# juliuspleunes4/TurboInfer

Measured on AMD Instinct MI355X. Metric: decode tokens/s/GPU, Llama-7B-shape INT4 @2048 ctx; % HBM-read roofline, higher is better.
Workload: dtype w4a16; 1 GPU; llama2-7b INT4 g128 decode, 1 stream(s)/GPU, KV 2048, replay at pos 2047; model=llama2-7b, global_batch=1, seq_len=2048, parallelism=replicas1 (request-sharded, no collectives)

## Files before the change

include/ti_hip.h:

```cpp
#ifndef TI_HIP_H
#define TI_HIP_H

#include <stddef.h>
#include <stdint.h>

#ifdef __cplusplus
extern "C" {
#endif

typedef void* ti_stream_t;

enum ti_status {
  TI_OK = 0,
  TI_ERR_ARG = 1,
  TI_ERR_HIP = 2,
  TI_ERR_UNSUPPORTED = 3,
  TI_ERR_NOMEM = 4,
  TI_ERR_NODEV = 5
};

const char* ti_last_error(void);

int ti_device_count(int* count);
int ti_init(int device);
// ... 111 lines not shown
                   int kv_heads, int head_dim, int splits, float* workspace, uint16_t* out,
                   ti_stream_t s);
int ti_attn_decode_packed(const float* q, const uint16_t* k_cache, const uint16_t* v_cache,
                          int64_t kv_stream_stride, int max_seq, const int32_t* pos, int M, int heads,
                          int kv_heads, int head_dim, int splits, float* workspace, uint16_t* out,
                          ti_stream_t s);
#ifndef TI_ATTN_MAX_PART_SPLITS
#define TI_ATTN_MAX_PART_SPLITS 8
#endif
int ti_attn_decode_partials(const float* q, const uint16_t* k_cache, const uint16_t* v_cache,
                            int64_t kv_stream_stride, int max_seq, const int32_t* pos, int M, int heads,
                            int kv_heads, int head_dim, int splits, uint16_t* part_o, float* part_ml,
                            ti_stream_t s);
int ti_attn_decode_f8(const float* q, const uint8_t* k_cache, const uint8_t* v_cache, int64_t kv_stream_stride,
                      int max_seq, const int32_t* pos, int M, int heads, int kv_heads, int head_dim, int splits,
                      float* workspace, uint16_t* out, ti_stream_t s);
int ti_attn_decode_packed_f8(const float* q, const uint8_t* k_cache, const uint8_t* v_cache,
                             int64_t kv_stream_stride, int max_seq, const int32_t* pos, int M, int heads,
                             int kv_heads, int head_dim, int splits, float* workspace, uint16_t* out,
                             ti_stream_t s);
int ti_attn_decode_partials_f8(const float* q, const uint8_t* k_cache, const uint8_t* v_cache,
                               int64_t kv_stream_stride, int max_seq, const int32_t* pos, int M, int heads,
                               int kv_heads, int head_dim, int splits, uint16_t* part_o, float* part_ml,
                               ti_stream_t s);
int ti_qkv_attn_partials(const void* tiles, const uint16_t* scales, int bits, const uint16_t* fx,
                         const float* ss_in, int n_ss, float eps, const float* rope_cs, const int32_t* pos,
                         uint16_t* k_cache, uint16_t* v_cache, int max_seq, int K, int heads, int kv_heads,
                         int head_dim, int splits, uint16_t* part_o, float* part_ml, void* xchg, ti_stream_t s);
size_t ti_qkv_attn_part_o_elems(int heads, int head_dim, int splits);
size_t ti_qkv_attn_part_ml_elems(int heads, int head_dim, int splits);
size_t ti_qkv_attn_xchg_bytes(int heads, int splits);
size_t ti_qkv_attn_error_offset(int heads, int splits);
int ti_qkv_attn_supported(int bits, int K, int heads, int kv_heads, int head_dim, int splits);
int ti_attn_prefill(const float* q, const uint16_t* k_cache, const uint16_t* v_cache, int max_seq,
                    const int32_t* pos, int M, int heads, int kv_heads, int head_dim, uint16_t* out,
                    ti_stream_t s);
int ti_attn_prefill_f8(const float* q, const uint8_t* k_cache, const uint8_t* v_cache, int max_seq,
                       const int32_t* pos, int M, int heads, int kv_heads, int head_dim, uint16_t* out,
                       ti_stream_t s);
size_t ti_attn_prefill_split_workspace_bytes(int M, int heads, int head_dim, int splits);
int ti_attn_prefill_split(const float* q, const uint16_t* k_cache, const uint16_t* v_cache, int max_seq,
                          const int32_t* pos, int M, int heads, int kv_heads, int head_dim, int splits,
                          float* workspace, uint16_t* out, ti_stream_t s);
int ti_attn_prefill_set_kernel(int mode);

int ti_gemm_kernel_name(int bits, int x_kind, int M, int N, int K, char* buf, int len);

uint64_t ti_gemm_onerow_epi_launches(void);

int ti_hbm_calibrate(size_t bytes, int reps, double* read_gbps, double* copy_gbps, ti_stream_t s);


typedef struct ti_step_args {
  const uint16_t* emb;
  float* h;
  int32_t hidden, M, vocab, in_stride, out_stride, placeholder_first;
  const int32_t* in_tokens;
  const int32_t* n_in;
  unsigned long long* argmax;
  int32_t* out_tokens;
  int32_t* pos;
  const int32_t* base_pos;
  const int32_t* step_ctr;
  const float* fold_w;
  uint16_t* fold_x;
  float* fold_ss;
// ... 57 lines not shown
```

turboinfer_amd/__init__.py:

```python
from __future__ import annotations

import ctypes as C
import os
import subprocess

import numpy as np

HERE = os.path.dirname(os.path.abspath(__file__))
ROOT = os.path.dirname(HERE)
LIB_PATH = os.environ.get("TI_LIB") or os.path.join(HERE, "lib", "libturboinfer_amd.so")

TI_OK = 0
X_F16, X_F32, X_F32_RMSNORM, X_F16_FOLDED, X_ATTN_SPLITS, X_F16_PACKED = 0, 1, 2, 3, 4, 5
ATTN_MAX_PART_SPLITS = 8
EPI_STORE_F32, EPI_STORE_F16, EPI_RESID_F32, EPI_SILU_MUL_F16, EPI_QKV_ROPE_KV, EPI_LOGITS_ARGMAX = range(6)
ARGMAX_SLOTS = 32
GEMM_MAX_ROWS = 1024
BITS_G32 = 32
BITS_AFF = 64
BITS_KV8 = 128
SCALE_GROUP, SCALE_TENSOR, SCALE_UNIT = 0, 1, 2
ROWS_CONCAT, ROWS_INTERLEAVE8 = 0, 1
(W_Q, W_K, W_V, W_O, W_GATE, W_UP, W_DOWN, W_LM_HEAD, V_ATTN_NORM, V_FFN_NORM, V_OUT_NORM, E_EMBED) = range(12)

# ... 40 lines not shown
                ("max_batch", C.c_int32), ("compat", C.c_int32), ("device", C.c_int32),
                ("attn_splits", C.c_int32)]


EXPORTED = [
    "ti_last_error", "ti_device_count", "ti_init", "ti_device_name", "ti_malloc", "ti_free", "ti_memcpy_h2d",
    "ti_memcpy_d2h", "ti_memcpy_d2d", "ti_memset", "ti_stream_create", "ti_stream_destroy", "ti_stream_sync",
    "ti_device_sync", "ti_event_create", "ti_event_destroy", "ti_event_record", "ti_event_elapsed_ms",
    "ti_wpack_tile_bytes", "ti_wpack_scale_bytes", "ti_wpack_host", "ti_wsynth_device", "ti_fill_uniform_f16",
    "ti_fill_uniform_f32", "ti_fill_kv_uniform", "ti_kv_copy_slots", "ti_gemm_wq_a16", "ti_gemm_lds_bytes", "ti_gemm_prepare",
    "ti_gemm_max_rows", "ti_gemm_packed_rows", "ti_gemm_packed_rows_for", "ti_gemm_tile_plan", "ti_rmsnorm_f16", "ti_rmsnorm_f16_packed", "ti_attn_decode_packed", "ti_attn_prefill", "ti_attn_prefill_set_kernel",
    "ti_attn_workspace_bytes", "ti_attn_decode", "ti_step_begin", "ti_matmul_f32", "ti_rms_norm_f32",
    "ti_rope_f32", "ti_silu_f32", "ti_relu_f32", "ti_add_f32", "ti_mul_f32", "ti_softmax_f32", "ti_attention_f32",
    "ti_argmax_f32", "ti_engine_create", "ti_engine_destroy", "ti_engine_get_stream", "ti_engine_memory", "ti_engine_set_tensor",
    "ti_engine_synth", "ti_engine_fill_kv", "ti_engine_generate", "ti_engine_step", "ti_engine_compat_step",
    "ti_engine_replay_prepare", "ti_engine_set_prefill", "ti_engine_replay_run", "ti_engine_sync", "ti_engine_last_tokens",
    "ti_engine_time_kernel", "ti_engine_stamp_steps", "ti_rope_table", "ti_sample_token", 
    "ti_gemm_grid", "ti_engine_set_fold",
    "ti_attn_decode_partials", "ti_sample_device", "ti_sample_step", "ti_engine_generate_sampled",
    "ti_engine_beam_search", "ti_engine_serve", 
    "ti_wpack_q_host", "ti_engine_set_tensor_q", "ti_sample_workspace_bytes", "ti_sample_device_ws",
    "ti_wpack_q1_host", "ti_engine_set_tensor_q1", "ti_epilogue_bytes",
    "ti_sample_step_ws", "ti_hbm_calibrate", "ti_gemm_kernel_name",
    "ti_gemm_fold_partials", "ti_engine_set_stop", "ti_engine_counters",
    "ti_qkv_attn_partials", "ti_qkv_attn_part_o_elems", "ti_qkv_attn_part_ml_elems", "ti_engine_set_qkv_attn",
    "ti_qkv_attn_xchg_bytes", "ti_qkv_attn_supported", "ti_qkv_attn_error_offset",
    "ti_logprob_rows", "ti_engine_score",
    "ti_attn_decode_f8", "ti_attn_decode_packed_f8", "ti_attn_decode_partials_f8", "ti_fill_kv_uniform_f8",
    "ti_attn_prefill_f8", "ti_engine_prefill_attn_name",
    "ti_engine_read_kv",
    "ti_attn_prefill_split", "ti_attn_prefill_split_workspace_bytes", "ti_lookahead_begin", "ti_lookahead_accept",
    "ti_engine_generate_lookahead",
    "ti_gemm_onerow_epi_launches",
]

_lib = None


def build(jobs: int = 8) -> None:
    subprocess.run(["make", "-s", "-C", ROOT, f"-j{jobs}", "all"], check=True)


def lib() -> C.CDLL:
    global _lib
    if _lib is None:
        if not os.path.exists(LIB_PATH):
            raise TiError(f"native library missing: {LIB_PATH} (run `make` or __graft_entry__.build())")
        L = C.CDLL(LIB_PATH)
        vp, i32, i64, u64, f32, sz = C.c_void_p, C.c_int, C.c_int64, C.c_uint64, C.c_float, C.c_size_t
        L.ti_last_error.restype = C.c_char_p
        L.ti_device_count.argtypes = [C.POINTER(C.c_int)]
        L.ti_init.argtypes = [i32]
        L.ti_device_name.argtypes = [i32, C.c_char_p, i32]
        L.ti_malloc.argtypes = [C.POINTER(vp), sz]
        L.ti_free.argtypes = [vp]
        for n in ("ti_memcpy_h2d", "ti_memcpy_d2h", "ti_memcpy_d2d"):
            getattr(L, n).argtypes = [vp, vp, sz, vp]
        L.ti_memset.argtypes = [vp, i32, sz, vp]
        L.ti_stream_sync.argtypes = [vp]
        L.ti_wpack_tile_bytes.argtypes = [i32, i32, i32]
        L.ti_wpack_tile_bytes.restype = sz
        L.ti_wpack_scale_bytes.argtypes = [i32, i32, i32]
        L.ti_wpack_scale_bytes.restype = sz
        L.ti_wpack_host.argtypes = [vp, i32, i32, i32, i32, i32, i32, i32, vp, vp]
        L.ti_wsynth_device.argtypes = [u64, C.c_uint32, i32, i32, i32, i32, i32, i32, vp, vp, vp]
        L.ti_fill_uniform_f16.argtypes = [u64, C.c_uint32, u64, f32, vp, vp]
# ... 67 lines not shown
            L.ti_qkv_attn_partials.argtypes = [vp, vp, i32, vp, vp, i32, f32, vp, vp, vp, vp, i32, i32, i32, i32,
                                               i32, i32, vp, vp, vp, vp]
            L.ti_qkv_attn_xchg_bytes.argtypes = [i32, i32]
            L.ti_qkv_attn_supported.argtypes = [i32, i32, i32, i32, i32, i32]
            L.ti_qkv_attn_xchg_bytes.restype = sz
            L.ti_qkv_attn_error_offset.argtypes = [i32, i32]
            L.ti_qkv_attn_error_offset.restype = sz
            L.ti_qkv_attn_part_o_elems.argtypes = [i32, i32, i32]
            L.ti_qkv_attn_part_o_elems.restype = sz
            L.ti_qkv_attn_part_ml_elems.argtypes = [i32, i32, i32]
            L.ti_qkv_attn_part_ml_elems.restype = sz
        if hasattr(L, "ti_engine_score"):
            L.ti_logprob_rows.argtypes = [vp, i32, i32, i32, vp, vp, vp, vp]
            L.ti_engine_score.argtypes = [vp, i32, vp, i32, i32, vp, vp, vp]
        if hasattr(L, "ti_attn_decode_f8"):
            for n in ("ti_attn_decode_f8", "ti_attn_decode_packed_f8", "ti_attn_decode_partials_f8"):
                getattr(L, n).argtypes = [vp, vp, vp, i64, i32, vp, i32, i32, i32, i32, i32, vp, vp, vp]
            L.ti_fill_kv_uniform_f8.argtypes = [u64, C.c_uint32, i32, i32, i32, i32, vp, vp]
            L.ti_engine_read_kv.argtypes = [vp, i32, i32, i32, i32, i32, vp]
        if hasattr(L, "ti_attn_prefill_f8"):
            L.ti_attn_prefill_f8.argtypes = [vp, vp, vp, i32, vp, i32, i32, i32, i32, vp, vp]
            L.ti_engine_prefill_attn_name.argtypes = [vp, i32, C.c_char_p, i32]
        if hasattr(L, "ti_engine_generate_lookahead"):
            L.ti_attn_prefill_split.argtypes = [vp, vp, vp, i32, vp, i32, i32, i32, i32, i32, vp, vp, vp]
            L.ti_attn_prefill_split_workspace_bytes.argtypes = [i32, i32, i32, i32]
            L.ti_attn_prefill_split_workspace_bytes.restype = sz
            L.ti_lookahead_begin.argtypes = [C.POINTER(LookaheadArgs), vp]
            L.ti_lookahead_accept.argtypes = [C.POINTER(LookaheadArgs), vp]
            L.ti_engine_generate_lookahead.argtypes = [vp, i32, vp, i32, i32, vp, i32, i32, i32, i32, vp,
                                                       C.POINTER(LookaheadStats)]
        if hasattr(L, "ti_gemm_onerow_epi_launches"):
            L.ti_gemm_onerow_epi_launches.argtypes = []
            L.ti_gemm_onerow_epi_launches.restype = u64
        L.ti_engine_compat_step.argtypes = [vp, i32, vp]
        L.ti_engine_replay_prepare.argtypes = [vp, i32, i32, i32]
        L.ti_engine_replay_run.argtypes = [vp, i32]
        L.ti_engine_sync.argtypes = [vp]
        L.ti_engine_last_tokens.argtypes = [vp, i32, vp]
        L.ti_engine_time_kernel.argtypes = [vp, i32, i32, i32, i32, C.POINTER(C.c_double), C.POINTER(C.c_double)]
        if hasattr(L, "ti_engine_stamp_steps"):
            L.ti_engine_stamp_steps.argtypes = [vp, i32, i32, vp, vp, C.POINTER(C.c_int)]
        L.ti_hbm_calibrate.argtypes = [sz, i32, C.POINTER(C.c_double), C.POINTER(C.c_double), vp]
        L.ti_gemm_kernel_name.argtypes = [i32, i32, i32, i32, i32, C.c_char_p, i32]
        L.ti_rope_table.argtypes = [vp, i32, i32, f32, vp]
        L.ti_sample_token.argtypes = [vp, i32, f32, i32, f32, f32, C.POINTER(C.c_int), C.POINTER(C.c_float)]
        _lib = L
    return _lib


def check(rc: int) -> None:
    if rc != TI_OK:
        raise TiError(f"ti error {rc}: {lib().ti_last_error().decode()}")


def device_count() -> int:
    n = C.c_int(0)
    check(lib().ti_device_count(C.byref(n)))
    return n.value


def init(device: int = 0) -> None:
    check(lib().ti_init(device))


def _ptr(a: np.ndarray) -> C.c_void_p:
    return C.c_void_p(a.ctypes.data)
# ... 311 lines not shown
```

turboinfer_amd/csrc/host/engine.cpp:

```cpp
#include <hip/hip_runtime.h>

#include <algorithm>
#include <atomic>
#include <cmath>
#include <queue>
#include <cstdio>
#include <cstdlib>
#include <cstring>
#include <map>
#include <utility>
#include <vector>

#include "ti_engine.h"
#include "ti_hip.h"

int ti_set_error(int code, const char* fmt, ...);
int ti_check_hip(hipError_t e, const char* what);

#define E_CHECK(expr, what)                                \
  do {                                                     \
    hipError_t _e = (expr);                                \
    if (_e != hipSuccess) return ti_check_hip(_e, what);   \
  } while (0)
#define TI_TRY(expr)                 \
// ... 1922 lines not shown
  if (!e || e->replay_M < 1 || steps < 1 || steps > 256 || cap < 1 || !info_out || !t_out || !n_launch)
    return ti_set_error(TI_ERR_ARG, "ti_engine_stamp_steps: call ti_engine_replay_prepare first; 1 <= steps <= 256, "
                        "cap >= 1");
  DeviceScope bind_(e);
  TI_TRY(ti_stream_sync(e->s));
  std::vector<int32_t> info, info2;
  TI_TRY(capture_stamped(e, 1, nullptr, {}, info, nullptr));
  const size_t n = info.size() / 3, nt = n * (size_t)steps;
  std::vector<size_t> offs(nt);
  size_t words = 0;
  for (size_t i = 0; i < nt; ++i) {
    offs[i] = words;
    words += (size_t)info[3 * (i % n) + 2] * kStampWords;
  }
  if (words == 0) return ti_set_error(TI_ERR_UNSUPPORTED, "ti_engine_stamp_steps: no stamped launch in the step");
  void* buf = nullptr;
  TI_TRY(ti_malloc(&buf, words * 8));
  unsigned long long* st = static_cast<unsigned long long*>(buf);
  hipGraphExec_t g = nullptr;
  int rc = capture_stamped(e, steps, st, offs, info2, &g);
  if (rc == TI_OK && (info2.size() != nt * 3 || !std::equal(info.begin(), info.end(), info2.begin())))
    rc = ti_set_error(TI_ERR_UNSUPPORTED, "ti_engine_stamp_steps: the two captures differ");
  std::vector<unsigned long long> h(words);
  for (int it = 0; rc == TI_OK && it < 2; ++it) {
    hipError_t he = hipMemsetAsync(st, 0, words * 8, e->s);
    if (he == hipSuccess) he = hipGraphLaunch(g, e->s);
    if (he == hipSuccess && it == 1) he = hipMemcpyAsync(h.data(), st, words * 8, hipMemcpyDeviceToHost, e->s);
    if (he == hipSuccess) he = hipStreamSynchronize(e->s);
    if (he != hipSuccess) rc = ti_check_hip(he, "ti_engine_stamp_steps: replay");
  }
  if (g) hipGraphExecDestroy(g);
  ti_free(buf);
  TI_TRY(rc);
  constexpr double kUs = 0.01;
  std::vector<double> acc(n * TI_STAMP_FIELDS, 0.0), first(nt, 0.0), last_end(nt, 0.0);
  for (size_t i = 0; i < nt; ++i) {
    const int wgs = info[3 * (i % n) + 2];
    if (wgs == 0) continue;
    unsigned long long f = ~0ull, le = 0, lent = 0;
    double wskew = 0.0;
    std::vector<unsigned long long> ends, cus;
    ends.reserve(wgs);
    double ph[6] = {0, 0, 0, 0, 0, 0}, sskew = 0.0;
    int sskew_n = 0;
    int phn[6] = {0, 0, 0, 0, 0, 0};
    for (int w = 0; w < wgs; ++w) {
      const unsigned long long* p = h.data() + offs[i] + (size_t)w * kStampWords;
      if (p[0]) {
        f = std::min(f, p[0]);
        lent = std::max(lent, p[0]);
      }
      if (p[15]) cus.push_back((p[15] & 0x7FFFFFFF00000000ull) | (p[15] & 0xFF00ull));
      unsigned long long smn = ~0ull, smx = 0;
      for (int k = 16; k < 24; ++k)
        if (p[k]) {
          smn = std::min(smn, p[k]);
          smx = std::max(smx, p[k]);
        }
      if (smx) {
        sskew += (double)(smx - smn);
        ++sskew_n;
      }
      unsigned long long mn = ~0ull, mx = 0;
      for (int k = 1; k <= 8; ++k)
        if (p[k]) {
          mn = std::min(mn, p[k]);
// ... 58 lines not shown
```

turboinfer_amd/csrc/kernels/qkv_attn.hip:

```cpp
#include <math.h>
#include <stdlib.h>

#include "attention_body.hpp"
#include "common.hpp"
#include "dequant.hpp"
#include "ti_hip.h"

namespace ti {

struct QkvAttnArgs {
  const u32x4* tiles;
  const uint16_t* scales;
  const uint16_t* fx;
  const float* ss;
  int n_ss;
  float eps;
  const float* rope_cs;
  const int32_t* pos;
  uint16_t* kc;
  uint16_t* vc;
  int max_seq, K, heads, kv_heads, kv_shift, splits, kv_tiles;
  int last_extra;
  float scale;
  uint16_t* part_o;
  float* part_ml;
  unsigned long long* xchg;
  unsigned long long* stamp;
  uint32_t* err;
  int drop;
};

constexpr int kQaWaves = 8, kQaThreads = kQaWaves * kWave;
#ifndef TI_QA_KV_RING
#define TI_QA_KV_RING 3
#endif
#ifndef TI_QA_ISSUE_BARRIER
#define TI_QA_ISSUE_BARRIER 0
#endif
#ifndef TI_QA_KVW_LATE
#define TI_QA_KVW_LATE 0
#endif
#ifndef TI_QA_KV_LATE
#define TI_QA_KV_LATE -1
#endif
constexpr int kQaSlot = 32;
constexpr int kQaMaxK = 4096;
constexpr int kQaMaxKv = 2;
constexpr unsigned kQaSpin = 1u << 16;

__device__ __forceinline__ float int4_x_prep_qa(f16x8& h) {
  const f16 s16 = (f16)0.0625f;
  h[2] *= s16; h[3] *= s16; h[6] *= s16; h[7] *= s16;
  const float lo = ((float)h[0] + (float)h[1]) + ((float)h[4] + (float)h[5]);
  const float hi = ((float)h[2] + (float)h[3]) + ((float)h[6] + (float)h[7]);
  return 1032.0f * lo + 1152.0f * hi;
}

__host__ __device__ inline int qa_kv_tile(int h, int s, int i, int heads, int splits, int kv_tiles) {
  const int j = h + heads * (splits - 1 - s) + heads * splits * i;
  return j < kv_tiles ? j : -1;
}

template <int BITS, int HD, int NQ, int NK>
__global__ __launch_bounds__(kQaThreads, 1) void qkv_attn_kernel(const QkvAttnArgs a) {
  const unsigned long long t_entry = stamp_now();
  constexpr int C = TileFmt<BITS>::kChunks;
  constexpr int QT = HD / 16;
  __shared__ __attribute__((aligned(16))) f16 xl[kQaMaxK + 8];
  __shared__ __attribute__((aligned(16))) uint16_t sl[1 + kQaMaxKv][kQaMaxK / 128][16];
  __shared__ __attribute__((aligned(16))) float corr[kQaMaxK / 128][16];
  __shared__ u32x4 sl_dummy;
  __shared__ float slab[1 + kQaMaxKv][kQaWaves][16];
  __shared__ float q_s[HD];
  __shared__ float s_m[kQaWaves], s_l[kQaWaves];
  __shared__ __attribute__((aligned(16))) float s_acc[kQaWaves][HD];

  const int tid = threadIdx.x, lane = tid & 63;
  const int wave = __builtin_amdgcn_readfirstlane(tid >> 6);
  const int S = a.splits, h = (int)blockIdx.x / S, s = (int)blockIdx.x % S;
  const int K = a.K, KT = K >> 7, K8 = K >> 3;
  const int qd = a.heads * HD, kvd = a.kv_heads * HD;
  const int kparts = S / QT, tq = s % QT, kp = s / QT;
  const int KTP = KT / kparts;
  int gk[kQaMaxKv], nkv = 0;
#pragma unroll
  for (int i = 0; i < kQaMaxKv; ++i) {
    const int j = qa_kv_tile(h, s, i, a.heads, S, a.kv_tiles);
    gk[i] = qd / 16 + (j >= 0 ? j : 0);
    nkv += j >= 0 ? 1 : 0;
  }
  const int gq = h * QT + tq;
  unsigned long long* my_slot = a.xchg + ((size_t)h * S + s) * kQaSlot;

  int zero;
  asm volatile("v_mov_b32 %0, 0" : "=v"(zero));
  const int p_v = a.pos[zero];
  const uint32_t gen_prev = ld_sc1_u32((const uint32_t*)(my_slot + (zero & 15)) + 1);
  const int n_scq = KTP * 2, n_sc = n_scq + nkv * KT * 2;
  u32x4 sc_reg;
  {
    const int ic = tid < n_sc ? tid : 0, r2 = ic - n_scq, ik = r2 >= KT * 2 ? 1 : 0;
    const int g = ic < n_scq ? gq : ik ? gk[1] : gk[0];
    const int piece = ic < n_scq ? kp * KTP * 2 + ic : r2 - ik * KT * 2;
    sc_reg = *((const u32x4*)(a.scales + (size_t)g * KT * 16) + piece);
  }
  const u32x4 xr0 = *(const u32x4*)(a.fx + 8 * (tid < K8 ? tid : K8 - 1));
  float ss4[4];
#pragma unroll
  for (int j = 0; j < 4; ++j) ss4[j] = a.ss[lane + 64 * j < a.n_ss ? lane + 64 * j : 0];
  asm volatile("" ::: "memory");
  if constexpr (HD == 128 && TI_QA_ISSUE_BARRIER) __builtin_amdgcn_s_barrier();
  u32x4 wq[NQ][C];
#pragma unroll
  for (int i = 0; i < NQ; ++i) {
    const u32x4* src = a.tiles + ((size_t)gq * KT + kp * KTP + wave + kQaWaves * i) * (kWave * C) + lane;
#pragma unroll
    for (int c = 0; c < C; ++c) wq[i][c] = *(src + c * kWave);
  }
  constexpr bool kKvwUniform = HD == 128;
  u32x4 wk[kQaMaxKv][NK][C];
  auto load_kv_weights = [&]() {
#pragma unroll
    for (int t = 0; t < kQaMaxKv; ++t)
#pragma unroll
      for (int i = 0; i < NK; ++i)
        if (kKvwUniform || t < nkv) {
          const u32x4* src = a.tiles + ((size_t)gk[t] * KT + wave + kQaWaves * i) * (kWave * C) + lane;
#pragma unroll
          for (int c = 0; c < C; ++c) wk[t][i][c] = __builtin_nontemporal_load(src + c * kWave);
        }
  };
  if constexpr (kKvwUniform && !TI_QA_KVW_LATE) load_kv_weights();
  asm volatile("" ::: "memory");
  u32x4 xr = xr0;
  if constexpr (kKvwUniform)
    asm volatile("" : "+v"(xr), "+v"(sc_reg), "+v"(ss4[0]), "+v"(ss4[1]), "+v"(ss4[2]), "+v"(ss4[3]));
  {
    f16x8 hx = __builtin_bit_cast(f16x8, xr);
    float part = 0.0f;
    if constexpr (BITS == 4) part = int4_x_prep_qa(hx);
    *(f16x8*)(xl + 8 * tid) = hx;
    if constexpr (BITS == 4) {
      part = group_sum<16>(part);
      if (tid < K8 && (lane & 15) == 0) corr[tid >> 4][0] = part;
    }
  }
  {
    const int r2 = tid - n_scq, ik = r2 >= KT * 2 ? 1 : 0;
    *(tid < n_scq ? (u32x4*)&sl[0][0][0] + (kp * KTP * 2 + tid)
                  : tid < n_sc ? (u32x4*)&sl[1 + ik][0][0] + (r2 - ik * KT * 2) : &sl_dummy) = sc_reg;
  }
  float rms;
  {
    float t = 0.0f;
#pragma unroll
    for (int j = 0; j < 4; ++j) t += lane + 64 * j < a.n_ss ? ss4[j] : 0.0f;
    t = group_sum<kWave>(t);
    rms = sqrtf(t / (float)K + a.eps);
  }
  asm volatile("s_waitcnt lgkmcnt(0)" ::: "memory");
  __builtin_amdgcn_s_barrier();
  asm volatile("" ::: "memory");
  STAMP_MARK(ph_staged);
  const int p = __builtin_amdgcn_readfirstlane(p_v);
  const unsigned gen = (unsigned)__builtin_amdgcn_readfirstlane((int)gen_prev) + 1u;

  float2 cs;
  {
    const int gkw = wave == 3 ? gk[1] : gk[0];
    const int d = tid < HD ? tid : ((gkw - qd / 16) * 16 + (tid & 15)) % HD;
    cs = *(const float2*)(a.rope_cs + (size_t)p * HD + (d & ~1));
  }

  if constexpr (!kKvwUniform && !TI_QA_KVW_LATE) load_kv_weights();


  constexpr int LPK = HD / 8, KPW = 64 / LPK, RA = TI_QA_KV_RING;
  const int dl = lane % LPK, kg = lane / LPK;
  const int L = p;
  const int chunk = (L + a.last_extra + S - 1) / S;
  const int s0 = min(L, s * chunk), s1 = s == S - 1 ? L : min(L, s0 + chunk);
  const int nslot = s1 > s0 ? (s1 - s0 + KPW - 1) / KPW : 0;
  const int atot = wave < nslot ? (nslot - wave + kQaWaves - 1) / kQaWaves : 0;
  const size_t kv_off = (size_t)(h >> a.kv_shift) * a.max_seq * HD;
  auto slot_key = [&](int i) { return s0 + (wave + kQaWaves * i) * KPW + kg; };
  int arj = 0;
  u32x4 kr[RA], vr[RA];
  auto arefill = [&](int q) {
    const int key = min(slot_key(arj < atot ? arj : max(atot - 1, 0)), max(s1 - 1, 0));
    ++arj;
    kr[q] = ld_kv((const u32x4*)(a.kc + kv_off + (size_t)key * HD + dl * 8));
    vr[q] = ld_kv((const u32x4*)(a.vc + kv_off + (size_t)key * HD + dl * 8));
  };
  constexpr bool kKvLate = TI_QA_KV_LATE < 0 ? HD == 128 : TI_QA_KV_LATE != 0;
  if constexpr (!kKvLate) {
#pragma unroll
    for (int q = 0; q < RA; ++q) arefill(q);
  }

  const int r = lane & 15, kq = lane >> 4;
  const f16* xrow = xl + kq * 32;
  uint32_t magic;
  asm volatile("v_mov_b32 %0, 0x64006400" : "=v"(magic));
  auto item = [&](const u32x4 (&w)[C], int kt, const uint16_t* scl, f32x4& acc) {
    f32x4 t = {0.0f, 0.0f, 0.0f, 0.0f};
#pragma unroll
    for (int s4 = 0; s4 < 4; ++s4) {
      const f16x8 bf = dequant_step<BITS>(w, s4, magic);
      const f16x8 af = *(const f16x8*)(xrow + kt * 128 + s4 * 8);
      t = __builtin_amdgcn_mfma_f32_16x16x32_f16(af, bf, t, 0, 0, 0);
    }
    if constexpr (BITS == 4) t -= *(const f32x4*)(&corr[kt][4 * kq]);
    const float sc = h2f(scl[kt * 16 + r]);
    acc[0] = fmaf(sc, t[0], acc[0]);
    acc[1] = fmaf(sc, t[1], acc[1]);
    acc[2] = fmaf(sc, t[2], acc[2]);
    acc[3] = fmaf(sc, t[3], acc[3]);
  };
  {
    f32x4 acc = {0.0f, 0.0f, 0.0f, 0.0f};
#pragma unroll
    for (int i = 0; i < NQ; ++i) item(wq[i], kp * KTP + wave + kQaWaves * i, &sl[0][0][0], acc);
    if (lane < 16) slab[0][wave][lane] = acc[0];
  }
  STAMP_MARK(ph_qdata);
  asm volatile("s_waitcnt lgkmcnt(0)" ::: "memory");
  __builtin_amdgcn_s_barrier();
  asm volatile("" ::: "memory");
  STAMP_MARK(ph_qpart);
#if TI_QA_KVW_LATE
  load_kv_weights();
#endif
  if constexpr (kKvLate) {
#pragma unroll
    for (int q = 0; q < RA; ++q) arefill(q);
  }
  if (wave == 0 && lane < 16 && (int)blockIdx.x != a.drop) {
    float v = slab[0][0][lane];
#pragma unroll
    for (int w = 1; w < kQaWaves; ++w) v += slab[0][w][lane];
    st_sc1_u64(my_slot + lane, ((unsigned long long)gen << 32) | __builtin_bit_cast(uint32_t, v));
  }
  if (nkv > 0) {
#pragma unroll
    for (int t = 0; t < kQaMaxKv; ++t)
      if (t < nkv) {
        f32x4 acc = {0.0f, 0.0f, 0.0f, 0.0f};
#pragma unroll
        for (int i = 0; i < NK; ++i) item(wk[t][i], wave + kQaWaves * i, &sl[1 + t][0][0], acc);
        if (lane < 16) slab[1 + t][wave][lane] = acc[0];
      }
    asm volatile("s_waitcnt lgkmcnt(0)" ::: "memory");
    __builtin_amdgcn_s_barrier();
    asm volatile("" ::: "memory");
  }
  STAMP_MARK(ph_kv);
  if (wave >= 2 && wave - 2 < nkv) {
    const int ik = wave - 2, n = lane & 15;
    float v = slab[1 + ik][0][n];
#pragma unroll
    for (int w = 1; w < kQaWaves; ++w) v += slab[1 + ik][w][n];
    v = v / rms;
    const float partner = lane_xor<1>(v);
    if (lane < 16) {
      const int ng = (ik ? gk[1] : gk[0]) * 16 + n;
      const bool is_k = ng < qd + kvd;
      float rr = v;
      if (is_k) {
        const int d = (ng - qd) % HD;
        rr = (d & 1) == 0 ? fmaf(-partner, cs.y, v * cs.x) : fmaf(v, cs.x, partner * cs.y);
      }
      const int c = ng - qd - (is_k ? 0 : kvd), kvh = c / HD, dd = c - kvh * HD;
      const uint16_t hv = f2h(rr);
      (is_k ? a.kc : a.vc)[((size_t)kvh * a.max_seq + p) * HD + dd] = hv;
      const uint32_t pair = (uint32_t)hv | (lane_xor_u32<1>((uint32_t)hv) << 16);
      if ((n & 1) == 0) st_sc1_u64(my_slot + 16 + ik * 8 + (n >> 1), ((unsigned long long)gen << 32) | pair);
    }
  }

  if (tid < HD) {
    const int d = tid, t = d >> 4, n = d & 15;
    float v = 0.0f;
    bool lost = false;
    for (int part = 0; part < kparts; ++part) {
      const unsigned long long* g = a.xchg + ((size_t)h * S + t + QT * part) * kQaSlot + n;
      unsigned long long x = ld_sc1_u64(g);
      unsigned spin = 0;
      while ((unsigned)(x >> 32) != gen && ++spin < kQaSpin) {
        __builtin_amdgcn_s_sleep(1);
        x = ld_sc1_u64(g);
      }
      lost |= spin >= kQaSpin;
      v += __builtin_bit_cast(float, (uint32_t)x);
    }
    if (lost) st_sc1_u32(a.err + (tid & 1), 1u);
    v = v / rms;
    const float partner = lane_xor<1>(v);
    const float rr = (d & 1) == 0 ? fmaf(-partner, cs.y, v * cs.x) : fmaf(v, cs.x, partner * cs.y);
    q_s[d] = rr;
  }
  asm volatile("s_waitcnt lgkmcnt(0)" ::: "memory");
  __builtin_amdgcn_s_barrier();
  asm volatile("" ::: "memory");
  STAMP_MARK(ph_gathered);

  constexpr int kNewWave = kQaWaves - 1;
  const bool new_key = s == S - 1 && wave == kNewWave;
  const unsigned long long* nk_base[2];
  {
    const int dl0 = lane % (HD / 8), jk = (h >> a.kv_shift) * (HD / 16) + (dl0 >> 1), hs = a.heads * S;
    const float inv_heads = __builtin_amdgcn_rcpf((float)a.heads);
#pragma unroll
    for (int kv = 0; kv < 2; ++kv) {
      const int j = jk + kv * (a.kv_tiles >> 1), i = j >= hs ? 1 : 0, r2 = j - i * hs;
      const int q2 = (int)(((float)r2 + 0.5f) * inv_heads);
      nk_base[kv] = a.xchg + (size_t)((r2 - q2 * a.heads) * S + (S - 1 - q2)) * kQaSlot + 16 + i * 8 + (dl0 & 1) * 4;
    }
  }

  float qf[8];
#pragma unroll
  for (int e = 0; e < 8; ++e) qf[e] = q_s[dl * 8 + e] * a.scale;
  float mrun = -INFINITY, lrun = 0.0f, oacc[8];
#pragma unroll
  for (int e = 0; e < 8; ++e) oacc[e] = 0.0f;
  int ci = 0;
  auto consume_key = [&](const u32x4& kv, const u32x4& vv, bool valid) {
    float kf[8], vf[8];
    unpack8(kv, kf);
    unpack8(vv, vf);
    float dq = 0.0f;
#pragma unroll
    for (int e = 0; e < 8; ++e) dq = fmaf(qf[e], kf[e], dq);
    dq = group_sum<LPK>(dq);
    const float sc = valid ? dq : -INFINITY;
    const float mn = fmaxf(mrun, sc);
    const float alpha = mrun == mn ? 1.0f : __expf(mrun - mn);
    const float pr = valid ? __expf(sc - mn) : 0.0f;
    lrun = fmaf(lrun, alpha, pr);
    mrun = mn;
#pragma unroll
    for (int e = 0; e < 8; ++e) oacc[e] = fmaf(pr, vf[e], oacc[e] * alpha);
  };
  auto consume = [&](const u32x4& kv, const u32x4& vv) {
    const bool valid = slot_key(ci) < s1;
    ++ci;
    consume_key(kv, vv, valid);
  };
  int a0 = 0;
  for (; a0 + RA <= atot; a0 += RA) {
#pragma unroll
    for (int q = 0; q < RA; ++q) {
      ring_pin(kr[q], vr[q], lrun);
      consume(kr[q], vr[q]);
      arefill(q);
    }
  }
  auto ring_tail = [&]() {
#pragma unroll
    for (int q = 0; q < RA; ++q)
      if (a0 + q < atot) consume(kr[q], vr[q]);
  };
  if (new_key) {
    const unsigned long long* gp[8];
#pragma unroll
    for (int e = 0; e < 8; ++e) gp[e] = nk_base[e >> 2] + (e & 3);
    unsigned long long nkg[8];
#pragma unroll
    for (int e = 0; e < 8; ++e) nkg[e] = ld_sc1_u64(gp[e]);
#pragma unroll
    for (int q = 0; q < RA; ++q) asm volatile("" : "+v"(kr[q]), "+v"(vr[q])::"memory");
    ring_tail();
    bool lost = false;
#pragma unroll
    for (int e = 0; e < 8; ++e) {
      unsigned spin = 0;
      while ((unsigned)(nkg[e] >> 32) != gen && ++spin < kQaSpin) {
        __builtin_amdgcn_s_sleep(1);
        nkg[e] = ld_sc1_u64(gp[e]);
      }
      lost |= spin >= kQaSpin;
    }
// ... 11 lines not shown
#pragma unroll
    for (int e = 0; e < 8; ++e) oacc[e] = groups_sum<LPK>(oacc[e] * f);
    mrun = mx;
    lrun = l;
  }
  STAMP_MARK(ph_attn);
  if (lane < LPK)
#pragma unroll
    for (int e = 0; e < 8; ++e) s_acc[wave][dl * 8 + e] = oacc[e];
  if (lane == 0) {
    s_m[wave] = mrun;
    s_l[wave] = lrun;
  }
  __syncthreads();
  if (tid < HD) {
    const int d = tid;
    float mx = s_m[0];
#pragma unroll
    for (int w = 1; w < kQaWaves; ++w) mx = fmaxf(mx, s_m[w]);
    float o = 0.0f, l = 0.0f;
    if (mx != -INFINITY) {
#pragma unroll
      for (int w = 0; w < kQaWaves; ++w) {
        const float f = s_m[w] == -INFINITY ? 0.0f : __expf(s_m[w] - mx);
        o = fmaf(f, s_acc[w][d], o);
        l = fmaf(f, s_l[w], l);
      }
    }
    const size_t rrow = (size_t)h * S + s;
    a.part_o[rrow * HD + d] = f2h(l > 0.0f ? o / l : 0.0f);
    if (d == 0) *(float2*)(a.part_ml + 2 * rrow) = make_float2(mx, l);
  }
  STAMP_MARK(ph_end);
  stamp_end(a.stamp, t_entry, ph_staged, ph_qdata, ph_qpart, ph_kv, ph_gathered, ph_attn, ph_end);
}

}

using namespace ti;

extern "C" size_t ti_qkv_attn_part_o_elems(int heads, int head_dim, int splits) {
  return (size_t)heads * head_dim * (size_t)(splits + 2);
}
extern "C" size_t ti_qkv_attn_part_ml_elems(int heads, int head_dim, int splits) {
  return (size_t)heads * 2 * (size_t)splits + (size_t)heads * head_dim;
}
static size_t qa_granule_bytes(int heads, int splits) { return (size_t)heads * splits * kQaSlot * 8; }
extern "C" size_t ti_qkv_attn_xchg_bytes(int heads, int splits) { return qa_granule_bytes(heads, splits) + 64; }
extern "C" size_t ti_qkv_attn_error_offset(int heads, int splits) { return qa_granule_bytes(heads, splits); }

static bool qa_has_kernel(int bits, int head_dim, int nq, int nk, bool kv_uniform) {
  if (head_dim == 64) return (bits == 4 || bits == 8) && ((nq == 1 && (nk == 1 || nk == 2)) || (nq == 2 && nk == 2));
  return head_dim == 128 && (bits == 4 || bits == 8) && nq == 4 && nk == 4 && kv_uniform;
}

extern "C" int ti_qkv_attn_supported(int bits, int K, int heads, int kv_heads, int head_dim, int splits) {
  if ((bits != 4 && bits != 8) || (head_dim != 64 && head_dim != 128) || K < 1024 || K > kQaMaxK || K % 128 ||
      heads * head_dim > 4096 || kv_heads < 1 || heads < kv_heads || heads % kv_heads || (heads / kv_heads) & (heads / kv_heads - 1))
    return 0;
  const int QT = head_dim / 16, KT = K / 128, kv_tiles = 2 * kv_heads * head_dim / 16;
  if (splits < QT || splits > TI_ATTN_MAX_PART_SPLITS || splits % QT || KT % (splits / QT) || (KT / (splits / QT)) % 8 ||
      kv_tiles > heads * splits * kQaMaxKv)
    return 0;
  return qa_has_kernel(bits, head_dim, KT / (splits / QT) / kQaWaves, KT / kQaWaves, kv_tiles == kQaMaxKv * heads * splits)
             ? 1 : 0;
}

extern "C" int ti_qkv_attn_partials(const void* tiles, const uint16_t* scales, int bits, const uint16_t* fx,
                                    const float* ss_in, int n_ss, float eps, const float* rope_cs, const int32_t* pos,
                                    uint16_t* k_cache, uint16_t* v_cache, int max_seq, int K, int heads, int kv_heads,
                                    int head_dim, int splits, uint16_t* part_o, float* part_ml, void* xchg,
                                    ti_stream_t stream) {
  if (!tiles || !scales || !fx || !ss_in || !rope_cs || !pos || !k_cache || !v_cache || !part_o || !part_ml || !xchg)
    return ti_set_error(TI_ERR_ARG, "ti_qkv_attn_partials: null pointer");
  if (bits != 4 && bits != 8)
    return ti_set_error(TI_ERR_UNSUPPORTED, "ti_qkv_attn_partials: bits %d (4 or 8)", bits);
  if (head_dim != 64 && head_dim != 128)
    return ti_set_error(TI_ERR_UNSUPPORTED, "ti_qkv_attn_partials: head_dim %d (64 or 128)", head_dim);
  const int QT = head_dim / 16, KT = K / 128;
  if (K < 1024 || K > kQaMaxK || K % 128 || n_ss < 1 || n_ss > 256 || max_seq < 1 || heads * head_dim > 4096)
    return ti_set_error(TI_ERR_ARG, "ti_qkv_attn_partials: K %d (1024..%d, %% 128), n_ss %d (1..256)", K, kQaMaxK, n_ss);
  int kv_shift = 0;
  while (kv_heads > 0 && (kv_heads << kv_shift) < heads) ++kv_shift;
  if (kv_heads < 1 || heads < kv_heads || (kv_heads << kv_shift) != heads)
    return ti_set_error(TI_ERR_UNSUPPORTED, "ti_qkv_attn_partials: heads %d / kv_heads %d (a power of two)", heads,
                        kv_heads);
// ... 17 lines not shown
  a.K = K;
  a.heads = heads;
  a.kv_heads = kv_heads;
  a.kv_shift = kv_shift;
  a.splits = splits;
  a.kv_tiles = kv_tiles;
  {
    const int tile_bytes = KT * 1024 * (bits / 4), key_bytes = 2 * head_dim * 2;
    static const int env = [] {
      const char* v = getenv("TI_QA_EXTRA");
      return v ? atoi(v) : -1;
    }();
    a.last_extra = env >= 0 ? env
                   : kv_tiles >= heads && kv_tiles < heads * splits ? 2 * tile_bytes / key_bytes
                   : kQaWaves * (64 / (head_dim / 8));
  }
  a.scale = 1.0f / sqrtf((float)head_dim);
  a.part_o = part_o;
  a.part_ml = part_ml;
  a.xchg = (unsigned long long*)xchg;
  a.err = (uint32_t*)((char*)xchg + qa_granule_bytes(heads, splits));
  {
    const char* v = getenv("TI_QA_DROP");
    a.drop = v ? atoi(v) : -1;
  }
  const int grid = heads * splits;
  a.stamp = ti_stamp_next(STAMP_ATTN, grid);
  hipStream_t s = (hipStream_t)stream;
  if (head_dim == 128 && kv_tiles != kQaMaxKv * heads * splits)
    return ti_set_error(TI_ERR_UNSUPPORTED, "ti_qkv_attn_partials: head_dim 128 needs %d k / v tiles per workgroup",
                        kQaMaxKv);
  const int nq = KT / (splits / QT) / kQaWaves, nk = KT / kQaWaves, key = nq * 10 + nk;
  const dim3 g(grid), blk(kQaThreads);
#define TI_QA_CASE(B, H, Q, KK)                                                          \
  if (bits == B && head_dim == H && key == Q * 10 + KK) {                                \
    hipLaunchKernelGGL((qkv_attn_kernel<B, H, Q, KK>), g, blk, 0, s, a);               \
    TI_LAUNCH_CHECK("qkv_attn_kernel");                                                  \
    return TI_OK;                                                                        \
  }
  TI_QA_CASE(8, 64, 1, 2)
  TI_QA_CASE(4, 64, 1, 2)
  TI_QA_CASE(8, 64, 1, 1)
  TI_QA_CASE(4, 64, 1, 1)
  TI_QA_CASE(8, 64, 2, 2)
  TI_QA_CASE(4, 64, 2, 2)
  TI_QA_CASE(4, 128, 4, 4)
  TI_QA_CASE(8, 128, 4, 4)
#undef TI_QA_CASE
  return ti_set_error(TI_ERR_UNSUPPORTED, "ti_qkv_attn_partials: no kernel for bits %d, head_dim %d, %d q / %d k-v items per wave",
                      bits, head_dim, nq, nk);
}
```

Measured before the change: 845.2 tokens/s.

## Defer V-projection tile into the first attention round of fused QKV-attention kernel

```diff
diff --git a/include/ti_hip.h b/include/ti_hip.h
--- a/include/ti_hip.h
+++ b/include/ti_hip.h
@@ -167,6 +167,7 @@
 size_t ti_qkv_attn_xchg_bytes(int heads, int splits);
 size_t ti_qkv_attn_error_offset(int heads, int splits);
 int ti_qkv_attn_supported(int bits, int K, int heads, int kv_heads, int head_dim, int splits);
+int ti_qkv_attn_v_deferred(int bits, int head_dim);
 int ti_attn_prefill(const float* q, const uint16_t* k_cache, const uint16_t* v_cache, int max_seq,
                     const int32_t* pos, int M, int heads, int kv_heads, int head_dim, uint16_t* out,
                     ti_stream_t s);
diff --git a/turboinfer_amd/__init__.py b/turboinfer_amd/__init__.py
--- a/turboinfer_amd/__init__.py
+++ b/turboinfer_amd/__init__.py
@@ -96,6 +96,7 @@
     "ti_attn_prefill_split", "ti_attn_prefill_split_workspace_bytes", "ti_lookahead_begin", "ti_lookahead_accept",
     "ti_engine_generate_lookahead",
     "ti_gemm_onerow_epi_launches",
+    "ti_qkv_attn_v_deferred",
 ]
 
 _lib = None
@@ -229,6 +230,8 @@
         if hasattr(L, "ti_gemm_onerow_epi_launches"):
             L.ti_gemm_onerow_epi_launches.argtypes = []
             L.ti_gemm_onerow_epi_launches.restype = u64
+        if hasattr(L, "ti_qkv_attn_v_deferred"):
+            L.ti_qkv_attn_v_deferred.argtypes = [i32, i32]
         L.ti_engine_compat_step.argtypes = [vp, i32, vp]
         L.ti_engine_replay_prepare.argtypes = [vp, i32, i32, i32]
         L.ti_engine_replay_run.argtypes = [vp, i32]
diff --git a/turboinfer_amd/csrc/host/engine.cpp b/turboinfer_amd/csrc/host/engine.cpp
--- a/turboinfer_amd/csrc/host/engine.cpp
+++ b/turboinfer_amd/csrc/host/engine.cpp
@@ -1978,6 +1978,17 @@
   if (g) hipGraphExecDestroy(g);
   ti_free(buf);
   TI_TRY(rc);
+  if (const char* raw = getenv("TI_STAMP_RAW")) {
+    if (FILE* f = fopen(raw, "wb")) {
+      const unsigned long long hdr[3] = {n, (unsigned long long)steps, (unsigned long long)kStampWords};
+      std::vector<unsigned long long> o64(offs.begin(), offs.end());
+      fwrite(hdr, 8, 3, f);
+      fwrite(info.data(), 4, 3 * n, f);
+      fwrite(o64.data(), 8, nt, f);
+      fwrite(h.data(), 8, words, f);
+      fclose(f);
+    }
+  }
   constexpr double kUs = 0.01;
   std::vector<double> acc(n * TI_STAMP_FIELDS, 0.0), first(nt, 0.0), last_end(nt, 0.0);
   for (size_t i = 0; i < nt; ++i) {
diff --git a/turboinfer_amd/csrc/kernels/qkv_attn.hip b/turboinfer_amd/csrc/kernels/qkv_attn.hip
--- a/turboinfer_amd/csrc/kernels/qkv_attn.hip
+++ b/turboinfer_amd/csrc/kernels/qkv_attn.hip
@@ -43,6 +43,9 @@
 #ifndef TI_QA_KV_LATE
 #define TI_QA_KV_LATE -1
 #endif
+#ifndef TI_QA_Q_NT
+#define TI_QA_Q_NT 0
+#endif
 constexpr int kQaSlot = 32;
 constexpr int kQaMaxK = 4096;
 constexpr int kQaMaxKv = 2;
@@ -61,8 +64,9 @@
   return j < kv_tiles ? j : -1;
 }
 
-template <int BITS, int HD, int NQ, int NK>
+template <int BITS, int HD, int NQ, int NK, bool VD = false>
 __global__ __launch_bounds__(kQaThreads, 1) void qkv_attn_kernel(const QkvAttnArgs a) {
+  static_assert(!VD || (HD == 128 && NK % NQ == 0), "the deferred v tile: head_dim 128 (a k and a v tile per workgroup)");
   const unsigned long long t_entry = stamp_now();
   constexpr int C = TileFmt<BITS>::kChunks;
   constexpr int QT = HD / 16;
@@ -115,7 +119,10 @@
   for (int i = 0; i < NQ; ++i) {
     const u32x4* src = a.tiles + ((size_t)gq * KT + kp * KTP + wave + kQaWaves * i) * (kWave * C) + lane;
 #pragma unroll
-    for (int c = 0; c < C; ++c) wq[i][c] = *(src + c * kWave);
+    for (int c = 0; c < C; ++c) {
+      if constexpr (HD == 128 && TI_QA_Q_NT) wq[i][c] = __builtin_nontemporal_load(src + c * kWave);
+      else wq[i][c] = *(src + c * kWave);
+    }
   }
   constexpr bool kKvwUniform = HD == 128;
   u32x4 wk[kQaMaxKv][NK][C];
@@ -130,7 +137,16 @@
           for (int c = 0; c < C; ++c) wk[t][i][c] = __builtin_nontemporal_load(src + c * kWave);
         }
   };
-  if constexpr (kKvwUniform && !TI_QA_KVW_LATE) load_kv_weights();
+  auto load_kv_tile = [&](int t) {
+#pragma unroll
+    for (int i = 0; i < NK; ++i) {
+      const u32x4* src = a.tiles + ((size_t)(t ? gk[1] : gk[0]) * KT + wave + kQaWaves * i) * (kWave * C) + lane;
+#pragma unroll
+      for (int c = 0; c < C; ++c) wk[t][i][c] = __builtin_nontemporal_load(src + c * kWave);
+    }
+  };
+  if constexpr (VD) load_kv_tile(0);
+  else if constexpr (kKvwUniform && !TI_QA_KVW_LATE) load_kv_weights();
   asm volatile("" ::: "memory");
   u32x4 xr = xr0;
   if constexpr (kKvwUniform)
@@ -173,6 +189,11 @@
   }
 
   if constexpr (!kKvwUniform && !TI_QA_KVW_LATE) load_kv_weights();
+  if constexpr (VD) {
+    asm volatile("" ::: "memory");
+    load_kv_tile(1);
+    asm volatile("" ::: "memory");
+  }
 
 
   constexpr int LPK = HD / 8, KPW = 64 / LPK, RA = TI_QA_KV_RING;
@@ -229,8 +250,92 @@
   asm volatile("" ::: "memory");
   STAMP_MARK(ph_qpart);
 #if TI_QA_KVW_LATE
-  load_kv_weights();
+  if constexpr (!VD) load_kv_weights();
 #endif
+  auto kv_epilogue = [&](int ik, bool is_k) {
+    const int n = lane & 15;
+    float v = slab[1 + ik][0][n];
+#pragma unroll
+    for (int w = 1; w < kQaWaves; ++w) v += slab[1 + ik][w][n];
+    v = v / rms;
+    const float partner = lane_xor<1>(v);
+    if (lane < 16) {
+      const int ng = (ik ? gk[1] : gk[0]) * 16 + n;
+      float rr = v;
+      if (is_k) {
+        const int d = (ng - qd) % HD;
+        rr = (d & 1) == 0 ? fmaf(-partner, cs.y, v * cs.x) : fmaf(v, cs.x, partner * cs.y);
+      }
+      const int c = ng - qd - (is_k ? 0 : kvd), kvh = c / HD, dd = c - kvh * HD;
+      const uint16_t hv = f2h(rr);
+      (is_k ? a.kc : a.vc)[((size_t)kvh * a.max_seq + p) * HD + dd] = hv;
+      const uint32_t pair = (uint32_t)hv | (lane_xor_u32<1>((uint32_t)hv) << 16);
+      if ((n & 1) == 0) st_sc1_u64(my_slot + 16 + ik * 8 + (n >> 1), ((unsigned long long)gen << 32) | pair);
+    }
+  };
+  auto publish_q = [&]() {
+    if (wave == 0 && lane < 16 && (int)blockIdx.x != a.drop) {
+      float v = slab[0][0][lane];
+#pragma unroll
+      for (int w = 1; w < kQaWaves; ++w) v += slab[0][w][lane];
+      st_sc1_u64(my_slot + lane, ((unsigned long long)gen << 32) | __builtin_bit_cast(uint32_t, v));
+    }
+  };
+  auto q_finish = [&](int d, float v) {
+    v = v / rms;
+    const float partner = lane_xor<1>(v);
+    q_s[d] = (d & 1) == 0 ? fmaf(-partner, cs.y, v * cs.x) : fmaf(v, cs.x, partner * cs.y);
+  };
+  unsigned long long ph_kv = 0, ph_kitems = 0, ph_first = 0, ph_vbar = 0;
+#define TI_QA_MARK(var) do { if (TI_STAMP_PHASES) var = stamp_now(); } while (0)
+  if constexpr (VD) {
+    constexpr int KP = NK / NQ;
+    asm volatile("" : "+v"(cs.x), "+v"(cs.y));
+    auto k_items = [&]() {
+      f32x4 acc = {0.0f, 0.0f, 0.0f, 0.0f};
+#pragma unroll
+      for (int i = 0; i < NK; ++i) item(wk[0][i], wave + kQaWaves * i, &sl[1][0][0], acc);
+      if (lane < 16) slab[1][wave][lane] = acc[0];
+    };
+    publish_q();
+    k_items();
+    TI_QA_MARK(ph_kitems);
+    const int d = tid & (HD - 1), t = d >> 4, n = d & 15;
+    const unsigned long long* g[KP];
+    unsigned long long x[KP];
+#pragma unroll
+    for (int part = 0; part < KP; ++part) {
+      g[part] = a.xchg + ((size_t)h * S + t + QT * part) * kQaSlot + n;
+      x[part] = ld_sc1_u64(g[part]);
+    }
+    asm volatile("" ::: "memory");
+#pragma unroll
+    for (int q = 0; q < RA; ++q) arefill(q);
+#pragma unroll
+    for (int part = 0; part < KP; ++part) asm volatile("" : "+v"(x[part])::"memory");
+    if (tid < HD) {
+      bool miss = false;
+#pragma unroll
+      for (int part = 0; part < KP; ++part) miss |= (unsigned)(x[part] >> 32) != gen;
+      if (__builtin_expect(miss, 0)) {
+        bool lost = false;
+#pragma unroll
+        for (int part = 0; part < KP; ++part) {
+          unsigned spin = 0;
+          while ((unsigned)(x[part] >> 32) != gen && ++spin < kQaSpin) {
+            __builtin_amdgcn_s_sleep(1);
+            x[part] = ld_sc1_u64(g[part]);
+          }
+          lost |= spin >= kQaSpin;
+        }
+        if (lost) st_sc1_u32(a.err + (tid & 1), 1u);
+      }
+      float v = 0.0f;
+#pragma unroll
+      for (int part = 0; part < KP; ++part) v += __builtin_bit_cast(float, (uint32_t)x[part]);
+      q_finish(d, v);
+    }
+  } else {
   if constexpr (kKvLate) {
 #pragma unroll
     for (int q = 0; q < RA; ++q) arefill(q);
@@ -254,7 +359,7 @@
     __builtin_amdgcn_s_barrier();
     asm volatile("" ::: "memory");
   }
-  STAMP_MARK(ph_kv);
+  TI_QA_MARK(ph_kv);
   if (wave >= 2 && wave - 2 < nkv) {
     const int ik = wave - 2, n = lane & 15;
     float v = slab[1 + ik][0][n];
@@ -299,10 +404,13 @@
     const float rr = (d & 1) == 0 ? fmaf(-partner, cs.y, v * cs.x) : fmaf(v, cs.x, partner * cs.y);
     q_s[d] = rr;
   }
+  }
   asm volatile("s_waitcnt lgkmcnt(0)" ::: "memory");
   __builtin_amdgcn_s_barrier();
   asm volatile("" ::: "memory");
   STAMP_MARK(ph_gathered);
+  if constexpr (VD)
+    if (wave == 2) kv_epilogue(0, true);
 
   constexpr int kNewWave = kQaWaves - 1;
   const bool new_key = s == S - 1 && wave == kNewWave;
@@ -348,6 +456,37 @@
     consume_key(kv, vv, valid);
   };
   int a0 = 0;
+  f32x4 vacc = {0.0f, 0.0f, 0.0f, 0.0f};
+  auto v_item = [&](int i) { item(wk[1][i], wave + kQaWaves * i, &sl[2][0][0], vacc); };
+  constexpr int kVps = 2, kVslots = (NK + kVps - 1) / kVps;
+  static_assert(!VD || kVslots <= RA, "the v items fit the first main round");
+  auto v_publish = [&]() {
+    if (lane < 16) slab[2][wave][lane] = vacc[0];
+    asm volatile("s_waitcnt lgkmcnt(0)" ::: "memory");
+    __builtin_amdgcn_s_barrier();
+    asm volatile("" ::: "memory");
+    TI_QA_MARK(ph_vbar);
+    if (wave == 3) kv_epilogue(1, false);
+  };
+  if constexpr (VD) {
+    if (RA <= atot) {
+#pragma unroll
+      for (int q = 0; q < RA; ++q) {
+        ring_pin(kr[q], vr[q], lrun);
+        consume(kr[q], vr[q]);
+        arefill(q);
+        if (q == 0) TI_QA_MARK(ph_first);
+#pragma unroll
+        for (int i = q * kVps; i < (q + 1) * kVps && i < NK; ++i) v_item(i);
+        if (q == kVslots - 1) v_publish();
+      }
+      a0 = RA;
+    } else {
+#pragma unroll
+      for (int i = 0; i < NK; ++i) v_item(i);
+      v_publish();
+    }
+  }
   for (; a0 + RA <= atot; a0 += RA) {
 #pragma unroll
     for (int q = 0; q < RA; ++q) {
@@ -425,7 +564,9 @@
     if (d == 0) *(float2*)(a.part_ml + 2 * rrow) = make_float2(mx, l);
   }
   STAMP_MARK(ph_end);
-  stamp_end(a.stamp, t_entry, ph_staged, ph_qdata, ph_qpart, ph_kv, ph_gathered, ph_attn, ph_end);
+  if constexpr (VD) stamp_end(a.stamp, t_entry, ph_staged, ph_kitems, ph_gathered, ph_first, ph_vbar, ph_attn, ph_end);
+  else stamp_end(a.stamp, t_entry, ph_staged, ph_qdata, ph_qpart, ph_kv, ph_gathered, ph_attn, ph_end);
+#undef TI_QA_MARK
 }
 
 }
@@ -445,6 +586,17 @@
 static bool qa_has_kernel(int bits, int head_dim, int nq, int nk, bool kv_uniform) {
   if (head_dim == 64) return (bits == 4 || bits == 8) && ((nq == 1 && (nk == 1 || nk == 2)) || (nq == 2 && nk == 2));
   return head_dim == 128 && (bits == 4 || bits == 8) && nq == 4 && nk == 4 && kv_uniform;
+}
+
+static bool qa_vdefer_knob() {
+  static const bool on = [] {
+    const char* v = getenv("TI_QA_VDEFER");
+    return v ? atoi(v) != 0 : true;
+  }();
+  return on;
+}
+extern "C" int ti_qkv_attn_v_deferred(int bits, int head_dim) {
+  return head_dim == 128 && (bits == 4 || bits == 8) && qa_vdefer_knob() ? 1 : 0;
 }
 
 extern "C" int ti_qkv_attn_supported(int bits, int K, int heads, int kv_heads, int head_dim, int splits) {
@@ -528,21 +680,26 @@
                         kQaMaxKv);
   const int nq = KT / (splits / QT) / kQaWaves, nk = KT / kQaWaves, key = nq * 10 + nk;
   const dim3 g(grid), blk(kQaThreads);
-#define TI_QA_CASE(B, H, Q, KK)                                                          \
-  if (bits == B && head_dim == H && key == Q * 10 + KK) {                                \
-    hipLaunchKernelGGL((qkv_attn_kernel<B, H, Q, KK>), g, blk, 0, s, a);               \
+  const bool vd = ti_qkv_attn_v_deferred(bits, head_dim) != 0;
+#define TI_QA_CASE_VD(B, H, Q, KK, V)                                                    \
+  if (bits == B && head_dim == H && key == Q * 10 + KK && vd == V) {                     \
+    hipLaunchKernelGGL((qkv_attn_kernel<B, H, Q, KK, V>), g, blk, 0, s, a);            \
     TI_LAUNCH_CHECK("qkv_attn_kernel");                                                  \
     return TI_OK;                                                                        \
   }
+#define TI_QA_CASE(B, H, Q, KK) TI_QA_CASE_VD(B, H, Q, KK, false)
   TI_QA_CASE(8, 64, 1, 2)
   TI_QA_CASE(4, 64, 1, 2)
   TI_QA_CASE(8, 64, 1, 1)
   TI_QA_CASE(4, 64, 1, 1)
   TI_QA_CASE(8, 64, 2, 2)
   TI_QA_CASE(4, 64, 2, 2)
+  TI_QA_CASE_VD(4, 128, 4, 4, true)
+  TI_QA_CASE_VD(8, 128, 4, 4, true)
   TI_QA_CASE(4, 128, 4, 4)
   TI_QA_CASE(8, 128, 4, 4)
 #undef TI_QA_CASE
+#undef TI_QA_CASE_VD
   return ti_set_error(TI_ERR_UNSUPPORTED, "ti_qkv_attn_partials: no kernel for bits %d, head_dim %d, %d q / %d k-v items per wave",
                       bits, head_dim, nq, nk);
 }
```

New measurement: 856.4 tokens/s, median of 6. 1.01x the previous value.
